# jan-frost/uzliti_slam

Hardware: AMD Instinct MI355X
Metric: SE(3) edges optimized/sec (node-pairs matched/sec in `secondary`) (higher is better)
Workload: dtype f64; 1 GPU; BASELINE config 2: 1000-node / 5000-edge SE(3) pose graph, 20 LM iterations, Huber(1) on loop closures; one independent graph per GPU; system_edges=4999

## Files before the change

uzliti_slam_amd/capi.py:

```python
import ctypes as C
import os
import subprocess

import numpy as np

_HERE = os.path.dirname(os.path.abspath(__file__))
LIB_PATH = os.environ.get("UZL_LIB", os.path.join(_HERE, "libuzl_mi355x.so"))
CSRC = os.path.join(_HERE, "csrc")

c_f64p = C.POINTER(C.c_double)
c_i32p = C.POINTER(C.c_int32)
c_u8p = C.POINTER(C.c_uint8)
c_u64p = C.POINTER(C.c_uint64)
c_i64p = C.POINTER(C.c_int64)

UZL_OK = 0
UZL_ERR_BAD_ARG = -1
UZL_ERR_NO_DEVICE = -2
UZL_ERR_HIP = -3
UZL_ERR_NOT_CONVERGED = -4
UZL_ERR_BUSY = -5
UZL_ERR_OOM = -6
UZL_ERR_NOT_FOUND = -7
UZL_ERR_STATE = -8
# ... 895 lines not shown
def ml_plan(row_ptr, col, precond_on=True, strong_blocks=False, mult_banned=False, comp4_off=False, arrays=True):
    rp = np.ascontiguousarray(row_ptr, np.int32); cl = np.ascontiguousarray(col, np.int32)
    nb = len(rp) - 1
    flags = C.c_int32((1 if precond_on else 0) | (2 if strong_blocks else 0) | (4 if mult_banned else 0) | (8 if comp4_off else 0))
    L = diag_lib()

    def call(level, what, info, out, nbytes):
        rc = L.uzl_debug_ml_plan(C.c_int32(nb), _p(rp, c_i32p), _p(cl, c_i32p), flags, C.c_int32(level), C.c_int32(what), _p(info, c_i32p),
                                 out.ctypes.data_as(C.c_void_p) if out is not None else None, C.byref(nbytes) if nbytes is not None else None)
        if rc != UZL_OK:
            raise UzlError(rc, "uzl_debug_ml_plan")

    def array(level, what):
        nbytes = C.c_int64(0)
        call(level, what, None, None, nbytes)
        out = np.zeros(nbytes.value // 4, np.int32)
        if nbytes.value:
            call(level, what, None, out, nbytes)
        return out

    info = np.zeros(64, np.int32)
    call(0, -1, info, None, None)
    out = dict(levels=int(info[0]), cl=int(info[1]), agg=int(info[2]), mult=int(info[3]), ns_steps=int(info[12]), gather_level=int(info[14]),
               lds=int(info[15]), rows=nb, lv=[])
    for l in range(out["levels"] + 1):
        lv = dict(n=int(info[16 + l]), fan=int(info[32 + l]), nslots=int(info[48 + l]))
        if arrays:
            lv["row_ptr"] = rp if l == 0 else array(l, 0)
            lv["col"] = cl if l == 0 else array(l, 1)
        out["lv"].append(lv)
    return out


class Radius(_Handle):

    _prefix, _cfg_type = "uzl_radius", RadiusCfg

    def set_nodes(self, poses, stamps_front_ns):
        P = np.ascontiguousarray(poses, np.float64).reshape(-1, 12); st = np.ascontiguousarray(stamps_front_ns, np.int64)
        self.n = len(P)
        self._check(lib().uzl_radius_set_nodes(self._h, C.c_int32(len(P)), _p(P, c_f64p), st.ctypes.data_as(C.POINTER(C.c_int64))))

    def query(self, queries, cap=None):
        q = np.ascontiguousarray(queries, np.int32)
        cap = int(cap if cap is not None else max(1, self.n * max(len(q), 1)))
        f = np.zeros(max(cap, 1), np.int32); t = np.zeros(max(cap, 1), np.int32); cnt = np.zeros(max(len(q), 1), np.int32)
        tot = C.c_int64()
        self._check(lib().uzl_radius_query(self._h, C.c_int32(len(q)), _p(q, c_i32p), C.c_int64(cap), _p(f, c_i32p), _p(t, c_i32p),
                                           _p(cnt, c_i32p), C.byref(tot)))
        w = min(tot.value, cap)
        return f[:w].copy(), t[:w].copy(), cnt[:len(q)].copy(), tot.value


class Places(_Handle):

    _prefix, _cfg_type = "uzl_places", PlacesCfg

    @staticmethod
    def _d(desc):
        d = np.ascontiguousarray(desc, np.uint8)
        return d, (d.shape[0] if d.ndim == 2 else 0), (d.shape[1] if d.ndim == 2 else 32)

    def search_and_add(self, desc, stamp_ns, cap=64):
        d, rows, nb = self._d(desc)
        out = np.zeros(max(cap, 1), np.int32); n = C.c_int32(); idx = C.c_int32()
        self._check(lib().uzl_places_search_and_add(self._h, _p(d, c_u8p) if rows else None, C.c_int32(rows), C.c_int32(nb), C.c_int64(int(stamp_ns)),
# ... 405 lines not shown
```

uzliti_slam_amd/csrc/pgo_handle.hpp:

```cpp
#pragma once
#include "uzl_common.hpp"
#include "pgo_types.hpp"
#include "pgo_schur.hpp"
#include "pgo_ml_plan.hpp"
#include "pgo_lm.hpp"

#include <algorithm>
#include <chrono>
#include <cstdlib>
#include <cmath>
#include <functional>
#include <limits>
#include <new>
#include <numeric>

namespace uzl {
void k_prepare_nodes(const uzl_node* nodes, int n, int xy, double* pose, hipStream_t s);
void k_prepare_flat_nodes(const double* poses12, int n, double* pose, hipStream_t s);
void k_prepare_edges(const uzl_edge* edges, const int32_t* src, int e, const double* sensors, int ns, int xy, int odom_params,
                     double* zinv, double* info, hipStream_t s);
void k_prepare_flat_edges(const double* meas12, const double* info36, int e, double* zinv, double* info, hipStream_t s);
int k_chi2(const PgoDev& D, const double* pose, double delta, hipStream_t s);
int k_chi2_trial(const PgoDev& D, const double* pose, double delta, hipStream_t s);
hipError_t k_hessian(const PgoDev& D, const double* pose, double delta, int* g_edges, int* g_rows, hipStream_t s, bool with_chi2 = true, hipEvent_t ev_a = nullptr,
// ... 3 lines not shown
void k_precond(const PgoDev& D, hipStream_t s);
void k_publish(const PgoDev& D, PgoHostScal* out_dev, uint32_t seq, hipStream_t s);
void k_set_scalar(double* dst, double v, hipStream_t s);
void k_set_scalar2(double* dst_a, double va, double* dst_b, double vb, hipStream_t s);
void k_residual_guard(const PgoDev& D, hipStream_t s);
void k_pcg_progress(const PgoDev& D, hipStream_t s);
void k_set_trial(double* scal, double lambda, double tol_f2, double eps_t, double eps_r, hipStream_t s);
int k_pcg_init(const PgoDev& D, double* p0, double* p1, hipStream_t s);
int k_pcg_spmv(const PgoDev& D, const double* p_old, double* p_new, int n_part, double tol2, hipStream_t s);
int k_pcg_update(const PgoDev& D, const double* p, int n_part, hipStream_t s);
int g_pcg_spmv(int nb);
int g_pcg_update(int nb);
int k_oplus(const PgoDev& D, const double* pose_in, double* pose_out, hipStream_t s);
int g_edges_for(int e);
void k_slot_records(const double* zinv, const double* info, int e, const int32_t* slot_edge, int nslots, double* srec, hipStream_t s);
int g_oplus_for(int n);
void k_edge_error(const PgoDev& D, const double* pose, double* err, hipStream_t s);
void k_poses_out(const double* pose, int n, double* out12, hipStream_t s);
void k_schur_gather(const PgoDev& D, const SchurDev& S, hipStream_t s);
void k_lm_head(const LmSlot* slots, int nslots, int pass_flags, hipStream_t s);
void k_lm_tail(const LmSlot* slots, int nslots, hipStream_t s);
hipError_t kl_linearize(const LmSlot* sl, int nslots, int g_edges, int g_asm, hipStream_t s);
void kl_eval(const LmSlot* sl, int nslots, int g_edges, int g_oplus, hipStream_t s);
void kl_schur_reduce(const LmSlot* sl, const LmShape& sh, hipStream_t s);
void kl_schur_backsub(const LmSlot* sl, const LmShape& sh, hipStream_t s);
void kl_schur_reduce(const HostSlot& hs, const LmShape& sh, hipStream_t s, KernelTimer* timer);
void kl_schur_backsub(const HostSlot& hs, const LmShape& sh, hipStream_t s, KernelTimer* timer);
void kl_ml_numeric(const LmSlot* sl, const LmShape& sh, int which, hipStream_t s);
void kl_ml_trial(const LmSlot* sl, const LmShape& sh, int which, int ns_steps, hipStream_t s);
void kl_ml_numeric(const HostSlot& hs, const LmShape& sh, hipStream_t s, KernelTimer* timer, const std::function<void()>& level1_done);
void kl_ml_trial(const HostSlot& hs, const LmShape& sh, int ns_steps, hipStream_t s, KernelTimer* timer);
void ml_cg_variant(const MlHot& ml, int agg, size_t lds_full, int32_t* variant, int32_t* comp_u, uint64_t* lds);
hipError_t kl_ml_init(const LmSlot* sl, const LmSlot* by_value, const LmShape& sh, int ix, hipStream_t s);
hipError_t kl_ml_pcg_its(const LmSlot* sl, const LmSlot* by_value, const LmShape& sh, int ix, double tol2, int first, int n, hipStream_t s, hipEvent_t* ev = nullptr);
void kl_ml_pcg_init(const HostSlot& hs, const LmShape& sh, hipStream_t s);
void kl_ml_spmv(const HostSlot& hs, const LmShape& sh, int parity, hipStream_t s, hipEvent_t ev_a = nullptr, hipEvent_t ev_b = nullptr);
hipError_t kl_ml_cg(const HostSlot& hs, const LmShape& sh, int parity, int init, hipStream_t s, hipEvent_t ev_a = nullptr, hipEvent_t ev_b = nullptr);
}



namespace uzl { struct LmRun; }
using namespace uzl;

struct SysBufs {
    DevBuf<int32_t> row_ptr, col, rowhdr, b2v;
    DevBuf<double> blk, hdiag, minv, x, xs, r, z, p, p2, ap;
    std::vector<int32_t> upload(int nb, const std::vector<int32_t>& h_row_ptr, const std::vector<int32_t>& h_col, const std::vector<int32_t>& h_b2v, hipStream_t s)
    {
        const int nslots = h_row_ptr[nb];
        const size_t nbz = std::max(nb, 1), nsz = std::max(nslots, 1);
        b2v.reserve(nbz); row_ptr.reserve(nbz + 1); col.reserve(nsz); rowhdr.reserve(nbz * kRowHdr);
        blk.reserve(nsz * 36);
        hdiag.reserve(nbz * 42); minv.reserve(nbz * 36);
        x.reserve(nbz * 6); xs.reserve(nbz * 6); r.reserve(nbz * 6); z.reserve(nbz * 6); p.reserve(nbz * 6); p2.reserve(nbz * 6);
        ap.reserve(nbz * 12 + kMaxPartials);
        std::vector<int32_t> hdr(nbz * kRowHdr, -1);
        for (int a = 0; a < nb; a++) {
            hdr[(size_t)a * kRowHdr] = h_row_ptr[a]; hdr[(size_t)a * kRowHdr + 1] = h_row_ptr[a + 1];
            for (int k = 0; k < 20 && h_row_ptr[a] + k < h_row_ptr[a + 1]; k++) hdr[(size_t)a * kRowHdr + 2 + k] = h_col[h_row_ptr[a] + k];
        }
        if (nb > 0) UZL_HIP(hipMemcpyAsync(b2v.p, h_b2v.data(), sizeof(int32_t) * nb, hipMemcpyHostToDevice, s));
        UZL_HIP(hipMemcpyAsync(row_ptr.p, h_row_ptr.data(), sizeof(int32_t) * (nb + 1), hipMemcpyHostToDevice, s));
        if (nslots > 0) UZL_HIP(hipMemcpyAsync(col.p, h_col.data(), sizeof(int32_t) * nslots, hipMemcpyHostToDevice, s));
        UZL_HIP(hipMemcpyAsync(rowhdr.p, hdr.data(), sizeof(int32_t) * hdr.size(), hipMemcpyHostToDevice, s));
        return hdr;
    }
// ... 139 lines not shown
```

uzliti_slam_amd/csrc/pgo_lm.hpp:

```cpp
#pragma once
#include <cmath>
#include <hip/hip_runtime.h>

#include "pgo_types.hpp"

namespace uzl {

#define UZL_HD __host__ __device__ __forceinline__

constexpr double kResidualGuard = 0.25;
constexpr double kRateDrop = 0.6;
constexpr double kTolFloor2 = 1e-4;
constexpr double kStepT = 1.0, kStepR = 0.1;

UZL_HD double lm_cube(double t)
{
#pragma clang fp contract(off)
    const double p = t * t, pe = fma(t, t, -p);
    const double q = p * t, qe = fma(p, t, -q);
    return q + (qe + pe * t);
}

UZL_HD double lm_log(double x)
{
// ... 1 lines not shown
    if (!(x < 1e300)) return 690.77552789821368;
    if (!(x > 1e-300)) return -690.77552789821368;
    int e = 0;
    double m = x;
    while (m >= 1.4142135623730951) { m *= 0.5; e++; }
    while (m < 0.70710678118654757) { m *= 2.0; e--; }
    const double s = (m - 1.) / (m + 1.), s2 = s * s;
    double term = s, sum = 0.;
    for (int k = 1; k < 60; k += 2) {
        sum += term / k;
        term *= s2;
        if (term < 1e-20 && term > -1e-20) break;
    }
    return 2. * sum + e * 0.69314718055994529;
}

UZL_HD double lm_pcg_rate(double rz_stop, double rz_end, int its, double tol2, double tol_f2)
{
#pragma clang fp contract(off)
    const double rz0 = rz_stop / (tol2 * tol_f2);
    return (its >= 16 && rz0 > 0. && rz_end > 0. && rz_end < rz0) ? lm_log(rz0 / rz_end) / its : -1.;
}

UZL_HD bool lm_refresh(int it, int iterations, bool may_run_last, double last_rel, double refresh_rel, double rate_ref, double rate_last,
                       double rate_drop = kRateDrop)
{
#pragma clang fp contract(off)
    return it == 0 || ((last_rel > refresh_rel || (rate_ref > 0. && rate_last > 0. && rate_last < rate_drop * rate_ref)) &&
                       (may_run_last || it + 1 < iterations));
}

UZL_HD int lm_pass_ix(int phase, int ix, int pending) { return (phase == kLmLin && pending) ? (ix ^ 1) : ix; }

struct LmStep { double rho; bool accepted; double last_rel; };
UZL_HD LmStep lm_step(double current_chi, double temp_chi, double scale_sum, double& lambda, double& ni)
{
#pragma clang fp contract(off)
    LmStep r;
    const double scale = scale_sum + 1e-3;
    r.rho = (current_chi - temp_chi) / scale;
    r.accepted = r.rho > 0 && std::isfinite(temp_chi);
    r.last_rel = 0.;
    if (r.accepted) {
        double alpha = 1. - lm_cube(2 * r.rho - 1);
        alpha = alpha < 2. / 3. ? alpha : 2. / 3.;
        const double scaleFactor = (1. / 3. > alpha) ? 1. / 3. : alpha;
        lambda *= scaleFactor;
        ni = 2.;
        const double at = temp_chi < 0 ? -temp_chi : temp_chi, d = current_chi - temp_chi;
        r.last_rel = (d < 0 ? -d : d) / (at > 1e-300 ? at : 1e-300);
    } else {
        lambda *= ni;
        ni *= 2.;
    }
    return r;
}

}
```

uzliti_slam_amd/csrc/pgo_ml_kernels.hip:

```cpp
#include <hip/hip_ext.h>
#include <functional>
#include <mutex>
#include <type_traits>

#include "pgo_device.hpp"
#include "uzl_common.hpp"

namespace uzl {

#ifdef UZL_STAMPS
__device__ unsigned long long g_stamps[64];
#define STAMP_DECL unsigned long long st_prev_ = __builtin_amdgcn_s_memrealtime(); int st_i_ = 0;
#define STAMP(base) do { if (blockIdx.x == 0 && threadIdx.x == 0) { unsigned long long n_ = __builtin_amdgcn_s_memrealtime(); \
        atomicAdd(&g_stamps[(base) + st_i_], n_ - st_prev_); st_prev_ = n_; } st_i_++; } while (0)
#else
#define STAMP_DECL
#define STAMP(base) do { } while (0)
#endif

struct P3 { double X[9], Y[9], Z[9]; };

__device__ __forceinline__ void mat3(const double* A, const double* B, double* C)
{
#pragma unroll
// ... 2399 lines not shown
    A.flags = D.flags; A.scal = D.scal; A.part_a = D.part_a; A.part_b = D.part_b; A.part_c = D.part_c;
    A.rowhdr = D.rowhdr; A.hdiag = D.hdiag; A.z = D.z; A.blk = D.blk; A.pbuf[0] = S.pbuf[0]; A.pbuf[1] = S.pbuf[1];
    A.r = D.r; A.x = D.x; A.xs = D.xs; A.ap = D.ap;
    A.geo0 = at(H.geo0); A.Winv0 = at(H.Winv[0]); A.Cmat32 = at(H.Cmat32); A.rg[0] = at(S.rg[0][0]); A.rg[1] = at(S.rg[0][1]);
    A.Sg = H.Sg; A.lm = lm; A.col = D.col; A.b = D.b; A.tol2 = tol2;
    A.nb = D.nb; A.n1 = H.n[1]; A.c32_stride = H.c32_stride; A.diag_owner = D.diag_owner;
    A.g_rows = S.g_rows; A.g_spmv = S.g_spmv; A.ix = ix;
    return A;
}
static void pcg_init(const PcgArgs& A, hipStream_t s) { hipLaunchKernelGGL(ml_init_pcg_kernel, dim3(A.g_rows), dim3(kCgBlk), 0, s, A); }
static void pcg_spmv(const PcgArgs& A, int parity, hipStream_t s, hipEvent_t ev_a = nullptr, hipEvent_t ev_b = nullptr)
{
    launch(ml_spmv_pcg_kernel, dim3(A.g_spmv), dim3(512), 0, s, ev_a, ev_b, A, parity);
}
static void pcg_cg(const PcgArgs& A, int comp_u, int parity, int init, hipStream_t s, hipEvent_t ev_a = nullptr, hipEvent_t ev_b = nullptr)
{
    auto pick = [&](auto k5, auto k8, auto k12, auto k16) { return comp_u <= 5 ? k5 : comp_u <= 8 ? k8 : comp_u <= 12 ? k12 : k16; };
    auto kernel = init ? pick(ml_cg_comp_pcg_kernel<5, true>, ml_cg_comp_pcg_kernel<8, true>, ml_cg_comp_pcg_kernel<12, true>, ml_cg_comp_pcg_kernel<16, true>)
                       : pick(ml_cg_comp_pcg_kernel<5, false>, ml_cg_comp_pcg_kernel<8, false>, ml_cg_comp_pcg_kernel<12, false>, ml_cg_comp_pcg_kernel<16, false>);
    launch(kernel, dim3(A.g_rows), dim3(kCgBlk), 0, s, ev_a, ev_b, A, parity);
}

hipError_t kl_ml_init(const LmSlot* sl, const LmSlot* by_value, const LmShape& sh, int ix, hipStream_t s)
{
    if (by_value && pcg_args_shape(sh)) {
        const PcgArgs A = make_pcg_args(*by_value, by_value->lm, ix, 0.);
        pcg_init(A, s); pcg_cg(A, sh.comp_u, 0, 1, s);
        return hipSuccess;
    }
    if (by_value && sh.nslots == 1) { kl_ml_init_t<LmSlot>(*by_value, sh, s); return kl_ml_cg_t<LmSlot>(*by_value, sh, 0, 1, s); }
    kl_ml_init_t<const LmSlot*>(sl, sh, s);
    return kl_ml_cg_t<const LmSlot*>(sl, sh, 0, 1, s);
}
hipError_t kl_ml_pcg_its(const LmSlot* sl, const LmSlot* by_value, const LmShape& sh, int ix, double tol2, int first, int n, hipStream_t s, hipEvent_t* ev)
{
    const bool one = by_value && sh.nslots == 1 && !ev;
    const bool args = one && pcg_args_shape(sh);
    const PcgArgs A = args ? make_pcg_args(*by_value, by_value->lm, ix, tol2) : PcgArgs{};
    for (int q = 0; q < n; q++) {
        const int par = (first + q) & 1;
        hipError_t e;
        if (args) { pcg_spmv(A, par, s); pcg_cg(A, sh.comp_u, par, 0, s); e = hipSuccess; }
        else if (ev) { kl_ml_spmv_t<const LmSlot*>(sl, sh, par, s, ev[4 * q], ev[4 * q + 1]); e = kl_ml_cg_t<const LmSlot*>(sl, sh, par, 0, s, ev[4 * q + 2], ev[4 * q + 3]); }
        else if (one) { kl_ml_spmv_t<LmSlot>(*by_value, sh, par, s); e = kl_ml_cg_t<LmSlot>(*by_value, sh, par, 0, s); }
        else { kl_ml_spmv_t<const LmSlot*>(sl, sh, par, s); e = kl_ml_cg_t<const LmSlot*>(sl, sh, par, 0, s); }
        if (e != hipSuccess) return e;
    }
    return hipSuccess;
}
void kl_ml_pcg_init(const HostSlot& hs, const LmShape& sh, hipStream_t s)
{
    if (pcg_args_shape(sh)) pcg_init(make_pcg_args(hs.S, nullptr, hs.ix, hs.tol2), s);
    else kl_ml_init_t<HostSlot>(hs, sh, s);
}
void kl_ml_spmv(const HostSlot& hs, const LmShape& sh, int parity, hipStream_t s, hipEvent_t ev_a, hipEvent_t ev_b)
{
    if (pcg_args_shape(sh)) pcg_spmv(make_pcg_args(hs.S, nullptr, hs.ix, hs.tol2), parity, s, ev_a, ev_b);
    else kl_ml_spmv_t<HostSlot>(hs, sh, parity, s, ev_a, ev_b);
}
hipError_t kl_ml_cg(const HostSlot& hs, const LmShape& sh, int parity, int init, hipStream_t s, hipEvent_t ev_a, hipEvent_t ev_b)
{
    if (pcg_args_shape(sh)) { pcg_cg(make_pcg_args(hs.S, nullptr, hs.ix, hs.tol2), sh.comp_u, parity, init, s, ev_a, ev_b); return hipSuccess; }
    return kl_ml_cg_t<HostSlot>(hs, sh, parity, init, s, ev_a, ev_b);
}

}

#ifdef UZL_STAMPS
extern "C" UZL_DIAG_EXPORT int uzl_debug_read_stamps(unsigned long long* out, int reset)
{
    if (hipMemcpyFromSymbol(out, HIP_SYMBOL(uzl::g_stamps), sizeof(unsigned long long) * 64) != hipSuccess) return -3;
    if (reset) { unsigned long long z[64] = {0}; if (hipMemcpyToSymbol(HIP_SYMBOL(uzl::g_stamps), z, sizeof(z)) != hipSuccess) return -3; }
    return 0;
}
#endif
// ... 53 lines not shown
```

uzliti_slam_amd/csrc/pgo_types.hpp:

```cpp
#pragma once
#include <cstdint>
#include "../../include/uzl_mi355x.h"

namespace uzl {
constexpr size_t kMlLdsLimit = (size_t)140 * 1024;
__host__ __device__ inline size_t ml_comp4_lds(int n2) { return (size_t)6 * (size_t)n2 * 8 + 64; }


constexpr int kMaxPartials = 8192;
constexpr int kProgressEvery = 2;
constexpr int kRowHdr = 24;

struct PgoDev {
    int32_t n, nb, e, nslots;
    int32_t e_begin, e_end;
    int32_t diag_owner;
    int32_t sibling0;
    double* pose;
    double* pose_trial;
    const int32_t* v2b;
    const int32_t* b2v;
    const int32_t* ei;
    const int32_t* ej;
    const double* zinv;
// ... 92 lines not shown
constexpr int kBatchMax = 256;
constexpr int kBatchLaneMin = 12;

constexpr int kSchurElim = 78;
constexpr int kSchurRunOut = 120;

struct SchurDev {
    int32_t n_runs, n_int, nbr, nslots_r;
    const int32_t* run_ptr;
    const int32_t* run_rows;
    const int32_t* slotP;
    const int32_t* slotN;
    const int32_t* endL;
    const int32_t* endR;
    const int32_t* sep_rows;
    const int32_t* rsrc;
    const int32_t* inc_ptr;
    const int32_t* inc;
    double* runblk;
    double* elim;
    double* runout;
};

enum LmPhase : int32_t {
    kLmLin = 0,
    kLmSolve = 1,
    kLmRetry = 2,
    kLmNeedSetup = 3,
    kLmDone = 4,
    kLmAnomaly = 5
};
enum LmNeed : int32_t { kNeedNumeric = 1, kNeedTrial = 2, kNeedRebuild = 4 };
enum LmPassFlags : int32_t { kPassSetup = 1 , kPassRebuild = 2  };
struct LmDev {
    int32_t flags[4];
    int32_t phase;
    int32_t cur;
    int32_t ix;
    int32_t pass;
    int32_t init_pass, schur_pass, numeric_pass, trial_pass;
    int32_t build_pass, build_ix, build_cur, need;
    int32_t it, qmax, iterations, max_it;
    int32_t pending, adopted, fresh, pcg_last;
    int32_t sync_rebuild, guarded, tails;
    int32_t st_pcg_iterations, st_lm_trials, st_precond_builds, st_iterations_done, st_terminated_early, anomaly_code, pad0;
    double lambda, ni, chi_cur, last_rel;
    double lambda_setup[2];
    double rate_ref, rate_last;
    double chi2_initial, tol_f2, eps_t, eps_r, refresh_rel, tol2, lambda_retake, delta;
    double scal2[8];
    double rate_drop;
};
struct LmHost {
    LmDev lm;
    double scal[8];
    uint32_t seq_begin, seq;
};
struct LmSlot {
    PgoDev D;
    PgoDev Dp;
    SchurDev SD;
    LmDev* lm;
    LmHost* pub;
    MlHot hot[2];
    const MlDev* dml[2];
    double* rg[2][2];
// ... 70 lines not shown
```

uzliti_slam_amd/csrc/uzl_pgo_lm.hip:

```cpp
#include "pgo_handle.hpp"

namespace uzl {

struct LmRun {
    int nslots = 0;
    DevBuf<LmSlot> d_slots;
    DevBuf<LmDev> d_lm;
    PinBuf<LmHost> h_pub;
    LmHost* d_pub = nullptr;
    PinBuf<LmDev> h_init;
    std::vector<LmSlot> slots;
    LmShape shape{};
    DevBuf<double> d_start;
    hipEvent_t ev_fork = nullptr, ev_join = nullptr;
    bool join_pending = false;
    uint64_t gen = ~0ull;
    int solves_of_gen = 0;
    int first_solve_its = 0;
    std::vector<std::vector<int>> trial_its_prev, trial_its_cur;
    std::vector<uint64_t> hist_gen;
    struct Seg { hipGraph_t g = nullptr; hipGraphExec_t x = nullptr; };
    Seg setup, reb, pcg_long[2];
    void drop(Seg& q) { if (q.x) { (void)hipGraphExecDestroy(q.x); q.x = nullptr; } if (q.g) { (void)hipGraphDestroy(q.g); q.g = nullptr; } }
    void drop_all() { drop(setup); drop(reb); drop(pcg_long[0]); drop(pcg_long[1]); }
// ... 18 lines not shown
        throw HipError{hipErrorUnknown, "hipEventCreate", __FILE__, __LINE__};
    }
    return R;
}
void reserve_slots(LmRun* R, int n)
{
    R->nslots = n;
    R->d_slots.reserve((size_t)n); R->d_lm.reserve((size_t)n);
    R->h_pub.reserve((size_t)n, hipHostMallocMapped | hipHostMallocCoherent);
    R->h_init.reserve((size_t)n);
    UZL_HIP(hipHostGetDevicePointer((void**)&R->d_pub, R->h_pub.p, 0));
    R->slots.resize((size_t)n);
}

void enq_linearize(LmRun* R, hipStream_t s)
{
    const LmShape& sh = R->shape;
    UZL_HIP(kl_linearize(R->d_slots.p, sh.nslots, sh.g_edges, sh.g_asm, s));
}
void enq_head(LmRun* R, int pass_flags, bool linearized, hipStream_t s)
{
    const LmShape& sh = R->shape;
    if (!linearized) enq_linearize(R, s);
    k_lm_head(R->d_slots.p, sh.nslots, pass_flags, s);
    if (sh.red) kl_schur_reduce(R->d_slots.p, sh, s);
}
void enq_setup(LmRun* R, int which, int ns_steps, hipStream_t s)
{
    kl_ml_numeric(R->d_slots.p, R->shape, which, s);
    kl_ml_trial(R->d_slots.p, R->shape, which, ns_steps, s);
}
const LmSlot* by_value_slot(LmRun* R) { return (R->shape.nslots == 1 && !R->shape.batch_geometry) ? R->slots.data() : nullptr; }
void enq_init(LmRun* R, int ix, hipStream_t s) { UZL_HIP(kl_ml_init(R->d_slots.p, by_value_slot(R), R->shape, ix, s)); }
void enq_pcg(LmRun* R, int ix, double tol2, int first, int n, hipStream_t s, hipEvent_t* ev = nullptr)
{
    UZL_HIP(kl_ml_pcg_its(R->d_slots.p, by_value_slot(R), R->shape, ix, tol2, first, n, s, ev));
}
void enq_tail(LmRun* R, hipStream_t s)
{
    const LmShape& sh = R->shape;
    if (sh.red) kl_schur_backsub(R->d_slots.p, sh, s);
    kl_eval(R->d_slots.p, sh.nslots, sh.g_edges, sh.g_oplus, s);
    k_lm_tail(R->d_slots.p, sh.nslots, s);
}
template <class F>
void run_seg(LmRun::Seg& q, bool eager, hipStream_t s, F&& enqueue)
{
    if (eager) { enqueue(s); return; }
    if (!q.x) {
        UZL_HIP(hipStreamBeginCapture(s, hipStreamCaptureModeThreadLocal));
        try { enqueue(s); }
        catch (...) {
            hipGraph_t part = nullptr;
            (void)hipStreamEndCapture(s, &part);
            if (part) (void)hipGraphDestroy(part);
            (void)hipGetLastError();
            throw;
        }
        UZL_HIP(hipStreamEndCapture(s, &q.g));
        UZL_HIP(hipGraphInstantiate(&q.x, q.g, nullptr, nullptr, 0));
    }
    UZL_HIP(hipGraphLaunch(q.x, s));
}

}

LmSlot make_slot(const uzl_pgo* h, LmDev* d_lm, LmHost* d_pub)
{
    LmSlot S;
// ... 150 lines not shown
        I.tails = (int32_t)sent[sl];
        R->h_init.p[sl] = I;
        UZL_HIP(hipMemcpyAsync(R->d_lm.p + sl, R->h_init.p + sl, sizeof(LmDev), hipMemcpyHostToDevice, s));
        memset(&snap[sl], 0, sizeof(LmHost));
        snap[sl].lm = I;
        solve_passes[sl] = 0; prev_last[sl] = 0; cur_last[sl] = 0; seen_trials[sl] = 0;
    };
    for (int sl = 0; sl < nS; sl++) load_slot(sl, true);
    R->join_pending = false;
    {
        bool same = R->hist_gen.size() == (size_t)Q;
        for (int j = 0; same && j < Q; j++) same = R->hist_gen[(size_t)j] == jobs[(size_t)j].h->structure_gen;
        if (same) R->trial_its_prev.swap(R->trial_its_cur); else R->trial_its_prev.clear();
        R->trial_its_prev.resize((size_t)Q);
        R->trial_its_cur.assign((size_t)Q, std::vector<int>());
        R->hist_gen.resize((size_t)Q);
        for (int j = 0; j < Q; j++) R->hist_gen[(size_t)j] = jobs[(size_t)j].h->structure_gen;
    }
    struct Drain {
        LmRun* R; hipStream_t s2;
        ~Drain() { if (R->join_pending) { (void)hipStreamSynchronize(s2); R->join_pending = false; } }
    } drain{R, o.s2};
    static const bool phases_on = diag_flag("UZL_PHASES");
    std::vector<hipEvent_t> ph_ev;
    std::vector<int> ph_tag;
    auto mark = [&](int tag) {
        if (!phases_on) return;
        hipEvent_t e; if (hipEventCreate(&e) != hipSuccess) return;
        (void)hipEventRecord(e, s); ph_ev.push_back(e); ph_tag.push_back(tag);
    };
    int passes = 0;
    double enq_ms = 0., wait_ms = 0.;
    bool lin_ahead = false;
    while (n_active > 0) {
        const auto tp0 = std::chrono::steady_clock::now();
        int pf = 0, want = 0;
        bool any_start = false;
        for (int sl = 0; sl < nS; sl++) {
            if (slot_job[sl] < 0 || jobs[slot_job[sl]].finished) continue;
            const LmDev& v = snap[sl].lm;
            int w;
            if (v.phase == kLmSolve) {
                w = solve_passes[sl] == 0 ? kStep : std::min(std::max(kStep, (v.flags[1] / 2 + 1) & ~1), 4 * kLong);
                solve_passes[sl]++;
            } else {
                any_start = true; solve_passes[sl] = 0;
                if (v.phase == kLmNeedSetup) pf |= ((v.need & (kNeedNumeric | kNeedTrial)) ? kPassSetup : 0) | ((v.need & kNeedRebuild) ? kPassRebuild : 0);
                else if (v.phase == kLmLin) {
                    if (lm_refresh(v.it, v.iterations, v.sync_rebuild != 0, v.last_rel, v.refresh_rel, v.rate_ref, v.rate_last, v.rate_drop))
                        pf |= (v.it == 0 || v.sync_rebuild) ? kPassSetup : kPassRebuild;
                    if (v.it > 0 && v.lambda > kLambdaRetake * v.lambda_setup[v.ix ^ (v.pending ? 1 : 0)]) pf |= kPassSetup;
                } else if (v.phase == kLmRetry) {
                    if (v.lambda > kLambdaRetake * v.lambda_setup[v.ix]) pf |= kPassSetup;
                }
                const bool no_history = jobs[(size_t)slot_job[sl]].h->cfg.pass_history == 1;
                auto up = [&](int count) { return nS == 1 ? count + 1 : ((count + 2) & ~1); };
                w = v.pcg_last > 0 ? up(v.pcg_last) : ((R->first_solve_its > 0 && !no_history) ? up(R->first_solve_its) : 2 * kLong);
                if (v.pcg_last > 0 && prev_last[sl] > 0 && v.pcg_last > prev_last[sl]) w = up(v.pcg_last + std::min(v.pcg_last - prev_last[sl], 16));
                {
                    const std::vector<int>& hist = R->trial_its_prev[(size_t)slot_job[sl]];
                    if (!no_history && (size_t)v.st_lm_trials < hist.size()) w = std::max(w, up(hist[(size_t)v.st_lm_trials]));
                }
                w = std::min(w, ((v.max_it + 1) & ~1));
            }
            want = std::max(want, w);
        }
        want = std::max(2, want);
        const int base = (nS == 1 && slot_job[0] >= 0 && snap[0].lm.phase == kLmSolve) ? snap[0].lm.flags[1] : 0;
        static const bool wrong_ix = diag_flag("UZL_LM_WRONG_IX");
        const int pass_ix = lm_pass_ix(snap[0].lm.phase, snap[0].lm.ix, snap[0].lm.pending) ^ (wrong_ix ? 1 : 0);
        const double tol2 = snap[0].lm.tol2;
        mark(0);
        if (any_start && R->join_pending) { UZL_HIP(hipStreamWaitEvent(s, R->ev_join, 0)); R->join_pending = false; }
        mark(1);
        if (any_start) enq_head(R, pf, lin_ahead, s);
        lin_ahead = false;
        mark(2);
        if (pf & kPassSetup) {
            const int steps = nS == 1 ? ml_ns_steps_at(R->shape.ns_steps, snap[0].lm.it) : R->shape.ns_steps;
            if (steps != R->shape.ns_steps) enq_setup(R, 1, steps, s);
            else run_seg(R->setup, eager, s, [&](hipStream_t q) { enq_setup(R, 1, steps, q); });
        }
        if (pf & kPassRebuild) {
            UZL_HIP(hipEventRecord(R->ev_fork, s));
            UZL_HIP(hipStreamWaitEvent(o.s2, R->ev_fork, 0));
            run_seg(R->reb, eager, o.s2, [&](hipStream_t q) { enq_setup(R, 0, R->shape.ns_steps, q); });
            UZL_HIP(hipEventRecord(R->ev_join, o.s2));
            R->join_pending = true;
        }
        mark(3);
        if (any_start) enq_init(R, pass_ix, s);
        mark(4);
        if (o.timer && o.timer->on) {
            std::vector<hipEvent_t> ev((size_t)4 * want);
            for (int q = 0; q < want; q++) { o.timer->pair(o.spmv_name, &ev[4 * q], &ev[4 * q + 1]); o.timer->pair(o.cg_name, &ev[4 * q + 2], &ev[4 * q + 3]); }
            enq_pcg(R, pass_ix, tol2, base, want, s, ev.data());
        } else {
            int first = base, left = want;
            if (!eager && (first & 1)) { enq_pcg(R, pass_ix, tol2, first, 1, s); first++; left--; }
            const int n_long = eager ? 0 : left / kLong, rem = left - n_long * kLong;
            for (int i = 0; i < n_long; i++) run_seg(R->pcg_long[pass_ix], false, s, [&](hipStream_t q) { enq_pcg(R, pass_ix, tol2, 0, kLong, q); });
            if (rem > 0) enq_pcg(R, pass_ix, tol2, first + n_long * kLong, rem, s);
        }
        mark(5);
        enq_tail(R, s);
        if (!R->join_pending && !(o.timer && o.timer->on)) { enq_linearize(R, s); lin_ahead = true; }
        mark(6);
        passes++;
        for (int sl = 0; sl < nS; sl++) sent[sl]++;
        const auto tp1 = std::chrono::steady_clock::now();
        if (o.verbose) fprintf(stderr, "[uzl_pgo]   pass %d enqueued: segments %d, %d PCG iterations, %d graph(s) in the slots\n", passes - 1, pf, want, n_active);
        bool refill = false;
        for (int sl = 0; sl < nS; sl++) {
            if (slot_job[sl] < 0 || jobs[slot_job[sl]].finished) continue;
            (void)wait_pub(s, R, sl, sent[sl], &snap[sl]);
            LmJob& J = jobs[slot_job[sl]];
            const LmDev& v = snap[sl].lm;
            J.passes++;
            if (o.verbose)
                fprintf(stderr, "[uzl_pgo] pass %d, graph %d -> it %d trial %d phase %d: pcg %d done %d (last solve %d) lambda %.3e chi2 %.9g |r|2/|b|2 %.3e need %d\n", passes - 1,
                        slot_job[sl], v.it, v.qmax, v.phase, v.flags[1], v.flags[0], v.pcg_last, v.lambda, v.chi_cur, snap[sl].scal[7], v.need);
            if (v.st_lm_trials > seen_trials[sl]) { seen_trials[sl] = v.st_lm_trials; prev_last[sl] = cur_last[sl]; cur_last[sl] = v.pcg_last; }
            if (v.st_lm_trials == 1 && v.pcg_last > 0 && slot_job[sl] == 0) R->first_solve_its = v.pcg_last;
            {
                std::vector<int>& cur = R->trial_its_cur[(size_t)slot_job[sl]];
                if (v.st_lm_trials > 0 && (size_t)v.st_lm_trials > cur.size()) cur.resize((size_t)v.st_lm_trials, v.pcg_last);
            }
            if (v.phase == kLmDone || v.phase == kLmAnomaly) {
                J.last = snap[sl]; J.finished = true; J.anomaly = v.phase == kLmAnomaly;
                n_active--; refill = true;
            }
        }
        if (o.timer && o.timer->on) { UZL_HIP(hipStreamSynchronize(s)); o.timer->resolve(); }
        if (refill && (n_active == 0 || nS == 1)) {
            if (R->join_pending && next_job < Q) { UZL_HIP(hipStreamWaitEvent(s, R->ev_join, 0)); R->join_pending = false; }
            for (int sl = 0; sl < nS; sl++)
                if (slot_job[sl] >= 0 && jobs[slot_job[sl]].finished) load_slot(sl, false);
            lin_ahead = false;
        }
        const auto tp2 = std::chrono::steady_clock::now();
        enq_ms += std::chrono::duration<double, std::milli>(tp1 - tp0).count(); wait_ms += std::chrono::duration<double, std::milli>(tp2 - tp1).count();
    }
    UZL_HIP(hipGetLastError());
    if (o.verbose) fprintf(stderr, "[uzl_pgo] device-resident loop: %d passes, host time enqueueing %.3f ms, waiting for snapshots %.3f ms\n", passes, enq_ms, wait_ms);
    if (R->join_pending) { UZL_HIP(hipStreamSynchronize(o.s2)); R->join_pending = false; }
    UZL_HIP(hipStreamSynchronize(s));
    if (phases_on && ph_ev.size() > 1) {
        double acc[7] = {0, 0, 0, 0, 0, 0, 0};
        static const char* nm[7] = {"wait for the rebuild (0->1)", "linearise + head (1->2)", "set-up / fork (2->3)", "init (3->4)", "pcg (4->5)", "tail (5->6)", "between passes (6->0)"};
        static const bool each = diag_flag("UZL_PHASES_EACH");
        for (size_t i = 0; i + 1 < ph_ev.size(); i++) {
            float ms = 0.f; (void)hipEventElapsedTime(&ms, ph_ev[i], ph_ev[i + 1]); acc[ph_tag[i] % 7] += ms;
            if (each) fprintf(stderr, "%s%d:%.0f", ph_tag[i] == 0 ? "\n[uzl_pgo]   " : " ", ph_tag[i], 1e3 * ms);
        }
        if (each) fprintf(stderr, "\n");
        fprintf(stderr, "[uzl_pgo] segments over %d passes (GPU event time, ms):", passes);
        for (int k = 0; k < 7; k++) fprintf(stderr, "  %s %.3f", nm[k], acc[k]);
        fprintf(stderr, "\n");
        for (hipEvent_t e : ph_ev) (void)hipEventDestroy(e);
    }
    return passes;
}

void finish_job(LmJob& J, uzl_pgo_stats* st, double wall_ms)
{
    uzl_pgo* h = J.h;
    const LmDev& v = J.last.lm;
    h->cur = v.cur ? h->pose_b.p : h->pose_a.p; h->trial = v.cur ? h->pose_a.p : h->pose_b.p;
    h->prev_pcg_iters = v.pcg_last;
    h->last_residual_ratio = J.last.scal[7];
    if (!st) return;
// ... 76 lines not shown
        R->drop_all();
        reserve_slots(R, nS);
        R->shape = sh;
    }
    std::vector<LmJob> jobs((size_t)Q);
    for (int g = 0; g < Q; g++) jobs[g].h = hs[g];
    LmDriveOpts o;
    o.s = s; o.s2 = s2; o.iterations = iterations; o.eager = eager || (timer && timer->on); o.verbose = verbose; o.timer = timer;
    o.spmv_name = "ml_spmv_batch"; o.cg_name = "ml_cg_comp_batch";
    lm_drive(R, jobs, o);
    const double wall = std::chrono::duration<double, std::milli>(std::chrono::steady_clock::now() - t0).count();
    int batched = 0;
    for (int g = 0; g < Q; g++) {
        LmJob& J = jobs[g];
        uzl_pgo* h = hs[g];
        static const int force_n = diag_int("UZL_BATCH_FORCE_ANOMALY_N", -1);
        if (!J.anomaly && h->n != force_n) { finish_job(J, stats ? stats + g : nullptr, wall); batched++; continue; }
        if (verbose) fprintf(stderr, "[uzl_pgo_batch] graph %d: anomaly %d at it %d trial %d -> single-graph path\n", g, J.last.lm.anomaly_code, J.last.lm.it, J.last.lm.qmax);
        UZL_HIP(hipMemcpyAsync(h->pose_a.p, R->d_start.p + J.start_off, sizeof(double) * 8 * (size_t)h->n, hipMemcpyDeviceToDevice, s));
        UZL_HIP(hipStreamSynchronize(s));
        h->cur = h->pose_a.p; h->trial = h->pose_b.p;
        own_streams(h, false);
        h->t_start = std::chrono::steady_clock::now();
        uzl_pgo_stats S;
        const int rc = do_optimize_host(h, iterations, &S);
        if (rc != UZL_OK && rc != UZL_ERR_NOT_CONVERGED) { *rc_all = rc; return -1 - g; }
        if (rc != UZL_OK) *rc_all = rc;
        if (stats) stats[g] = S;
    }
    return batched;
}

}
```

Before: 18.87 million edges/s.

## Split PCG iterations across passes by ending on SpMV and resuming with CG

In single-graph solves with by-value PCG args, each pass now ends with the next iteration's SpMV already issued, and the following pass begins with only the matching CG half. The aim is to keep the GPU busy while the host reads the snapshot between passes, hiding part of the per-pass latency. The pass planning logic moves into a pure function, exposed through a diagnostic hook for testing. It adds state (half_open) carried across passes, which must stay in step with the device iteration count, parity and the refill logic.

```diff
diff --git a/uzliti_slam_amd/capi.py b/uzliti_slam_amd/capi.py
--- a/uzliti_slam_amd/capi.py
+++ b/uzliti_slam_amd/capi.py
@@ -951,6 +951,23 @@
     return out
 
 
+LM_PASS_IN = ("nslots", "args", "timer", "eager", "k_long", "any_start", "pf", "lin_ahead", "solving", "its", "half_open", "want", "max_it", "join_pending")
+LM_PASS_PLAN = ("wait_join_head", "linearize", "lead_cg", "first", "pre", "n_long", "rem_first", "rem", "end_spmv", "n_spmv", "n_cg", "lin_ahead", "half_open",
+                "join_pending")
+
+
+def lm_pass_plan(**fields):
+    unknown = set(fields) - set(LM_PASS_IN)
+    if unknown:
+        raise TypeError("lm_pass_plan: unknown field(s) %s" % sorted(unknown))
+    a = np.array([int(fields.get(k, 0)) for k in LM_PASS_IN], np.int32)
+    out = np.zeros(len(LM_PASS_PLAN), np.int32)
+    rc = diag_lib().uzl_debug_lm_pass_plan(_p(a, c_i32p), _p(out, c_i32p))
+    if rc != UZL_OK:
+        raise UzlError(rc, "uzl_debug_lm_pass_plan")
+    return {k: int(v) for k, v in zip(LM_PASS_PLAN, out)}
+
+
 class Radius(_Handle):
 
     _prefix, _cfg_type = "uzl_radius", RadiusCfg
diff --git a/uzliti_slam_amd/csrc/pgo_handle.hpp b/uzliti_slam_amd/csrc/pgo_handle.hpp
--- a/uzliti_slam_amd/csrc/pgo_handle.hpp
+++ b/uzliti_slam_amd/csrc/pgo_handle.hpp
@@ -59,7 +59,9 @@
 void kl_ml_trial(const HostSlot& hs, const LmShape& sh, int ns_steps, hipStream_t s, KernelTimer* timer);
 void ml_cg_variant(const MlHot& ml, int agg, size_t lds_full, int32_t* variant, int32_t* comp_u, uint64_t* lds);
 hipError_t kl_ml_init(const LmSlot* sl, const LmSlot* by_value, const LmShape& sh, int ix, hipStream_t s);
-hipError_t kl_ml_pcg_its(const LmSlot* sl, const LmSlot* by_value, const LmShape& sh, int ix, double tol2, int first, int n, hipStream_t s, hipEvent_t* ev = nullptr);
+bool kl_pcg_args_shape(const LmSlot* by_value, const LmShape& sh);
+hipError_t kl_ml_pcg_its(const LmSlot* sl, const LmSlot* by_value, const LmShape& sh, int ix, double tol2, int first, int n, hipStream_t s, hipEvent_t* ev = nullptr,
+                         int halves = 0);
 void kl_ml_pcg_init(const HostSlot& hs, const LmShape& sh, hipStream_t s);
 void kl_ml_spmv(const HostSlot& hs, const LmShape& sh, int parity, hipStream_t s, hipEvent_t ev_a = nullptr, hipEvent_t ev_b = nullptr);
 hipError_t kl_ml_cg(const HostSlot& hs, const LmShape& sh, int parity, int init, hipStream_t s, hipEvent_t ev_a = nullptr, hipEvent_t ev_b = nullptr);
diff --git a/uzliti_slam_amd/csrc/pgo_lm.hpp b/uzliti_slam_amd/csrc/pgo_lm.hpp
--- a/uzliti_slam_amd/csrc/pgo_lm.hpp
+++ b/uzliti_slam_amd/csrc/pgo_lm.hpp
@@ -57,6 +57,46 @@
 
 UZL_HD int lm_pass_ix(int phase, int ix, int pending) { return (phase == kLmLin && pending) ? (ix ^ 1) : ix; }
 
+struct LmPassIn {
+    int32_t nslots, args, timer, eager, k_long;
+    int32_t any_start, pf, lin_ahead;
+    int32_t solving, its, half_open, want, max_it;
+    int32_t join_pending;
+};
+struct LmPassPlan {
+    int32_t wait_join_head, linearize;
+    int32_t lead_cg, first;
+    int32_t pre, n_long, rem_first, rem, end_spmv;
+    int32_t n_spmv, n_cg;
+    int32_t lin_ahead;
+    int32_t half_open, join_pending;
+};
+inline LmPassPlan lm_pass_plan(const LmPassIn& in)
+{
+    LmPassPlan P = {};
+    int join = in.join_pending;
+    if (in.any_start) {
+        P.wait_join_head = join;
+        P.linearize = in.lin_ahead ? 0 : 1;
+        join = (in.pf & kPassRebuild) ? 1 : 0;
+    }
+    const bool goes_on = in.nslots == 1 && !in.any_start && in.solving;
+    const int want = in.want > 2 ? in.want : 2;
+    P.lead_cg = (goes_on && in.half_open) ? 1 : 0;
+    P.first = goes_on ? in.its + P.lead_cg : 0;
+    P.end_spmv = (in.nslots == 1 && in.args && !in.timer && P.first + want < in.max_it) ? 1 : 0;
+    int i = P.first, left = want - P.end_spmv;
+    if (!in.eager && !in.timer && (i & 1) && left > 0) { P.pre = 1; i++; left--; }
+    P.n_long = (in.eager || in.timer || in.k_long <= 0) ? 0 : left / in.k_long;
+    P.rem_first = i + P.n_long * in.k_long;
+    P.rem = left - P.n_long * in.k_long;
+    P.n_spmv = want; P.n_cg = P.lead_cg + want - P.end_spmv;
+    P.half_open = P.end_spmv;
+    P.lin_ahead = (!in.timer && !join) ? 1 : 0;
+    P.join_pending = join;
+    return P;
+}
+
 struct LmStep { double rho; bool accepted; double last_rel; };
 UZL_HD LmStep lm_step(double current_chi, double temp_chi, double scale_sum, double& lambda, double& ni)
 {
diff --git a/uzliti_slam_amd/csrc/pgo_ml_kernels.hip b/uzliti_slam_amd/csrc/pgo_ml_kernels.hip
--- a/uzliti_slam_amd/csrc/pgo_ml_kernels.hip
+++ b/uzliti_slam_amd/csrc/pgo_ml_kernels.hip
@@ -2455,15 +2455,21 @@
     kl_ml_init_t<const LmSlot*>(sl, sh, s);
     return kl_ml_cg_t<const LmSlot*>(sl, sh, 0, 1, s);
 }
-hipError_t kl_ml_pcg_its(const LmSlot* sl, const LmSlot* by_value, const LmShape& sh, int ix, double tol2, int first, int n, hipStream_t s, hipEvent_t* ev)
+bool kl_pcg_args_shape(const LmSlot* by_value, const LmShape& sh) { return by_value && pcg_args_shape(sh); }
+hipError_t kl_ml_pcg_its(const LmSlot* sl, const LmSlot* by_value, const LmShape& sh, int ix, double tol2, int first, int n, hipStream_t s, hipEvent_t* ev, int halves)
 {
     const bool one = by_value && sh.nslots == 1 && !ev;
     const bool args = one && pcg_args_shape(sh);
+    if (halves && !args) return hipErrorInvalidValue;
     const PcgArgs A = args ? make_pcg_args(*by_value, by_value->lm, ix, tol2) : PcgArgs{};
     for (int q = 0; q < n; q++) {
         const int par = (first + q) & 1;
         hipError_t e;
-        if (args) { pcg_spmv(A, par, s); pcg_cg(A, sh.comp_u, par, 0, s); e = hipSuccess; }
+        if (args) {
+            if (!(q == 0 && (halves & kPcgBeginCg))) pcg_spmv(A, par, s);
+            if (!(q == n - 1 && (halves & kPcgEndSpmv))) pcg_cg(A, sh.comp_u, par, 0, s);
+            e = hipSuccess;
+        }
         else if (ev) { kl_ml_spmv_t<const LmSlot*>(sl, sh, par, s, ev[4 * q], ev[4 * q + 1]); e = kl_ml_cg_t<const LmSlot*>(sl, sh, par, 0, s, ev[4 * q + 2], ev[4 * q + 3]); }
         else if (one) { kl_ml_spmv_t<LmSlot>(*by_value, sh, par, s); e = kl_ml_cg_t<LmSlot>(*by_value, sh, par, 0, s); }
         else { kl_ml_spmv_t<const LmSlot*>(sl, sh, par, s); e = kl_ml_cg_t<const LmSlot*>(sl, sh, par, 0, s); }
diff --git a/uzliti_slam_amd/csrc/pgo_types.hpp b/uzliti_slam_amd/csrc/pgo_types.hpp
--- a/uzliti_slam_amd/csrc/pgo_types.hpp
+++ b/uzliti_slam_amd/csrc/pgo_types.hpp
@@ -148,6 +148,7 @@
 };
 enum LmNeed : int32_t { kNeedNumeric = 1, kNeedTrial = 2, kNeedRebuild = 4 };
 enum LmPassFlags : int32_t { kPassSetup = 1 , kPassRebuild = 2  };
+enum PcgHalves : int32_t { kPcgBeginCg = 1, kPcgEndSpmv = 2 };
 struct LmDev {
     int32_t flags[4];
     int32_t phase;
diff --git a/uzliti_slam_amd/csrc/uzl_pgo_lm.hip b/uzliti_slam_amd/csrc/uzl_pgo_lm.hip
--- a/uzliti_slam_amd/csrc/uzl_pgo_lm.hip
+++ b/uzliti_slam_amd/csrc/uzl_pgo_lm.hip
@@ -74,9 +74,9 @@
 }
 const LmSlot* by_value_slot(LmRun* R) { return (R->shape.nslots == 1 && !R->shape.batch_geometry) ? R->slots.data() : nullptr; }
 void enq_init(LmRun* R, int ix, hipStream_t s) { UZL_HIP(kl_ml_init(R->d_slots.p, by_value_slot(R), R->shape, ix, s)); }
-void enq_pcg(LmRun* R, int ix, double tol2, int first, int n, hipStream_t s, hipEvent_t* ev = nullptr)
-{
-    UZL_HIP(kl_ml_pcg_its(R->d_slots.p, by_value_slot(R), R->shape, ix, tol2, first, n, s, ev));
+void enq_pcg(LmRun* R, int ix, double tol2, int first, int n, hipStream_t s, hipEvent_t* ev = nullptr, int halves = 0)
+{
+    UZL_HIP(kl_ml_pcg_its(R->d_slots.p, by_value_slot(R), R->shape, ix, tol2, first, n, s, ev, halves));
 }
 void enq_tail(LmRun* R, hipStream_t s)
 {
@@ -293,6 +293,8 @@
     int passes = 0;
     double enq_ms = 0., wait_ms = 0.;
     bool lin_ahead = false;
+    bool half_open = false;
+    const bool pcg_args = kl_pcg_args_shape(by_value_slot(R), sh);
     while (n_active > 0) {
         const auto tp0 = std::chrono::steady_clock::now();
         int pf = 0, want = 0;
@@ -302,7 +304,8 @@
             const LmDev& v = snap[sl].lm;
             int w;
             if (v.phase == kLmSolve) {
-                w = solve_passes[sl] == 0 ? kStep : std::min(std::max(kStep, (v.flags[1] / 2 + 1) & ~1), 4 * kLong);
+                const int had = v.flags[1] + ((nS == 1 && half_open) ? 1 : 0);
+                w = solve_passes[sl] == 0 ? kStep : std::min(std::max(kStep, (had / 2 + 1) & ~1), 4 * kLong);
                 solve_passes[sl]++;
             } else {
                 any_start = true; solve_passes[sl] = 0;
@@ -327,14 +330,22 @@
             want = std::max(want, w);
         }
         want = std::max(2, want);
-        const int base = (nS == 1 && slot_job[0] >= 0 && snap[0].lm.phase == kLmSolve) ? snap[0].lm.flags[1] : 0;
         static const bool wrong_ix = diag_flag("UZL_LM_WRONG_IX");
         const int pass_ix = lm_pass_ix(snap[0].lm.phase, snap[0].lm.ix, snap[0].lm.pending) ^ (wrong_ix ? 1 : 0);
         const double tol2 = snap[0].lm.tol2;
+        const bool timed = o.timer && o.timer->on;
+        static const bool whole_pairs = diag_flag("UZL_LM_WHOLE_PAIRS");
+        LmPassIn in = {};
+        in.nslots = nS; in.args = (pcg_args && !whole_pairs) ? 1 : 0; in.timer = timed ? 1 : 0; in.eager = eager ? 1 : 0; in.k_long = kLong;
+        in.any_start = any_start ? 1 : 0; in.pf = pf; in.lin_ahead = lin_ahead ? 1 : 0;
+        in.solving = (nS == 1 && slot_job[0] >= 0 && snap[0].lm.phase == kLmSolve) ? 1 : 0;
+        in.its = snap[0].lm.flags[1]; in.half_open = half_open ? 1 : 0; in.want = want; in.max_it = snap[0].lm.max_it;
+        in.join_pending = R->join_pending ? 1 : 0;
+        const LmPassPlan P = lm_pass_plan(in);
         mark(0);
-        if (any_start && R->join_pending) { UZL_HIP(hipStreamWaitEvent(s, R->ev_join, 0)); R->join_pending = false; }
+        if (P.wait_join_head) { UZL_HIP(hipStreamWaitEvent(s, R->ev_join, 0)); R->join_pending = false; }
         mark(1);
-        if (any_start) enq_head(R, pf, lin_ahead, s);
+        if (any_start) enq_head(R, pf, !P.linearize, s);
         lin_ahead = false;
         mark(2);
         if (pf & kPassSetup) {
@@ -352,20 +363,19 @@
         mark(3);
         if (any_start) enq_init(R, pass_ix, s);
         mark(4);
-        if (o.timer && o.timer->on) {
+        if (timed) {
             std::vector<hipEvent_t> ev((size_t)4 * want);
             for (int q = 0; q < want; q++) { o.timer->pair(o.spmv_name, &ev[4 * q], &ev[4 * q + 1]); o.timer->pair(o.cg_name, &ev[4 * q + 2], &ev[4 * q + 3]); }
-            enq_pcg(R, pass_ix, tol2, base, want, s, ev.data());
+            enq_pcg(R, pass_ix, tol2, P.first, want, s, ev.data());
         } else {
-            int first = base, left = want;
-            if (!eager && (first & 1)) { enq_pcg(R, pass_ix, tol2, first, 1, s); first++; left--; }
-            const int n_long = eager ? 0 : left / kLong, rem = left - n_long * kLong;
-            for (int i = 0; i < n_long; i++) run_seg(R->pcg_long[pass_ix], false, s, [&](hipStream_t q) { enq_pcg(R, pass_ix, tol2, 0, kLong, q); });
-            if (rem > 0) enq_pcg(R, pass_ix, tol2, first + n_long * kLong, rem, s);
+            if (P.lead_cg) enq_pcg(R, pass_ix, tol2, P.first - 1, 1, s, nullptr, kPcgBeginCg);
+            if (P.pre) enq_pcg(R, pass_ix, tol2, P.first, 1, s);
+            for (int i = 0; i < P.n_long; i++) run_seg(R->pcg_long[pass_ix], false, s, [&](hipStream_t q) { enq_pcg(R, pass_ix, tol2, 0, kLong, q); });
+            if (P.rem + P.end_spmv > 0) enq_pcg(R, pass_ix, tol2, P.rem_first, P.rem + P.end_spmv, s, nullptr, P.end_spmv ? kPcgEndSpmv : 0);
         }
         mark(5);
         enq_tail(R, s);
-        if (!R->join_pending && !(o.timer && o.timer->on)) { enq_linearize(R, s); lin_ahead = true; }
+        if (P.lin_ahead) { enq_linearize(R, s); lin_ahead = true; }
         mark(6);
         passes++;
         for (int sl = 0; sl < nS; sl++) sent[sl]++;
@@ -387,6 +397,7 @@
                 std::vector<int>& cur = R->trial_its_cur[(size_t)slot_job[sl]];
                 if (v.st_lm_trials > 0 && (size_t)v.st_lm_trials > cur.size()) cur.resize((size_t)v.st_lm_trials, v.pcg_last);
             }
+            if (nS == 1) half_open = P.half_open && v.phase == kLmSolve;
             if (v.phase == kLmDone || v.phase == kLmAnomaly) {
                 J.last = snap[sl]; J.finished = true; J.anomaly = v.phase == kLmAnomaly;
                 n_active--; refill = true;
@@ -398,6 +409,7 @@
             for (int sl = 0; sl < nS; sl++)
                 if (slot_job[sl] >= 0 && jobs[slot_job[sl]].finished) load_slot(sl, false);
             lin_ahead = false;
+            half_open = false;
         }
         const auto tp2 = std::chrono::steady_clock::now();
         enq_ms += std::chrono::duration<double, std::milli>(tp1 - tp0).count(); wait_ms += std::chrono::duration<double, std::milli>(tp2 - tp1).count();
@@ -540,3 +552,16 @@
 }
 
 }
+
+#ifdef UZL_DIAG
+extern "C" UZL_DIAG_EXPORT int uzl_debug_lm_pass_plan(const int32_t* in, int32_t* out)
+{
+    static_assert(sizeof(uzl::LmPassIn) == 14 * sizeof(int32_t) && sizeof(uzl::LmPassPlan) == 14 * sizeof(int32_t), "the hook's words are the structs' fields");
+    if (!in || !out) return -1;
+    uzl::LmPassIn I;
+    memcpy(&I, in, sizeof(I));
+    const uzl::LmPassPlan P = uzl::lm_pass_plan(I);
+    memcpy(out, &P, sizeof(P));
+    return 0;
+}
+#endif
```

Result: no change. 18.74 million edges/s (-0.7%).
